# shaunliewsmu/ai-laryngeal-video-based-classifier

Hardware: AMD Instinct MI355X
Metric: clips/sec fwd ViViT-B 32x224^2 bf16 (higher is better)
Workload: dtype bf16; 1 GPU; ViViT-B/16x2 forward, 32x224x224 clips, batch 8 per GPU (BASELINE configs[1]); model=ViViT-B/16x2 (joint space-time, 12L, d768, 12H, 3137 tokens), global_batch=8, seq_len=3137, parallelism=dp1, streams=2, hip_graph=True

## Files before the change

ai-laryngeal-video-based-classifier_amd/_lib.py:

```python
from __future__ import annotations

import ctypes
import os
import re

import torch

from .build import LIB_PATH, INCLUDE

_lib = None

c_i64 = ctypes.c_int64
c_int = ctypes.c_int
c_f = ctypes.c_float
c_p = ctypes.c_void_p

SIGNATURES = {
    "vc_version": ([], ctypes.c_char_p),
    "vc_last_error": ([], ctypes.c_char_p),
    "vc_frame_gather": ([c_p, c_i64, c_i64, c_i64, c_i64, c_i64, c_p, c_i64, c_int, c_f, c_f, c_p, c_p], c_int),
    "vc_tubelet_im2col": ([c_p, c_i64, c_i64, c_i64, c_i64, c_i64, c_int, c_int, c_int, c_p, c_i64, c_p], c_int),
    "vc_patch_im2col": ([c_p, c_i64, c_i64, c_i64, c_i64, c_i64, c_int, c_int, c_int, c_int, c_int, c_p, c_i64, c_p],
                        c_int),
    "vc_layernorm_f32": ([c_p, c_i64, c_i64, c_i64, c_p, c_p, c_f, c_p, c_i64, c_p], c_int),
    "vc_gemm_bf16": ([c_p, c_i64, c_p, c_i64, c_i64, c_i64, c_i64, c_p, c_int, c_p, c_i64, c_p, c_i64,
                      c_i64, c_i64, c_i64, c_p], c_int),
    "vc_gemm_bf16_cfg": ([c_p, c_i64, c_p, c_i64, c_i64, c_i64, c_i64, c_p, c_int, c_p, c_i64, c_p, c_i64,
                          c_i64, c_i64, c_i64, c_int, c_p], c_int),
    "vc_layernorm_f32_bf16": ([c_p, c_i64, c_i64, c_i64, c_p, c_p, c_f, c_p, c_i64, c_p], c_int),
    "vc_attention_fwd": ([c_p, c_i64, c_i64, c_i64, c_i64, c_i64, c_f, c_int, c_p, c_i64, c_p], c_int),
    "vc_attention_fwd_rebase_always": ([c_p, c_i64, c_i64, c_i64, c_i64, c_f, c_p, c_i64, c_p], c_int),
    "vc_patch_im2col_h16": ([c_p, c_i64, c_i64, c_i64, c_i64, c_i64, c_int, c_int, c_int, c_int, c_int, c_int, c_p,
                             c_i64, c_p], c_int),
    "vc_gemm_pick": ([c_i64, c_i64, c_i64, c_int, c_i64, c_i64, c_p], c_int),
    "vc_gemm_h16_wrap": ([c_p, c_i64, c_i64, c_p, c_i64, c_i64, c_i64, c_i64, c_p, c_int, c_p, c_i64, c_p, c_i64,
                          c_i64, c_i64, c_i64, c_int, c_p], c_int),
    "vc_patch_im2col_split_h16": ([c_p, c_i64, c_i64, c_i64, c_i64, c_i64, c_int, c_int, c_int, c_int, c_int, c_int,
                                   c_p, c_i64, c_p], c_int),
    "vc_gemm_h16": ([c_p, c_i64, c_p, c_i64, c_i64, c_i64, c_i64, c_p, c_int, c_p, c_i64, c_p, c_i64,
                     c_i64, c_i64, c_i64, c_int, c_int, c_p], c_int),
    "vc_layernorm_f32_h16": ([c_p, c_i64, c_i64, c_i64, c_p, c_p, c_f, c_int, c_p, c_i64, c_p], c_int),
    "vc_attention_fwd_h16": ([c_p, c_i64, c_i64, c_i64, c_i64, c_i64, c_f, c_int, c_int, c_p, c_i64, c_p], c_int),
    "vc_spin": ([c_i64, c_i64, c_p], c_int),
    "vc_cls_init": ([c_p, c_p, c_p, c_i64, c_i64, c_i64, c_i64, c_p], c_int),
    "vc_cls_head": ([c_p, c_i64, c_i64, c_i64, c_i64, c_p, c_p, c_f, c_p, c_p, c_i64, c_p, c_p], c_int),
    "vc_temporal_attention": ([c_p, c_i64, c_i64, c_i64, c_i64, c_i64, c_i64, c_f, c_int, c_p, c_i64, c_p], c_int),
    "vc_window_attention3d": ([c_p, c_i64, c_i64, c_i64, c_i64, c_i64, c_i64, c_i64, c_int, c_int, c_int, c_int, c_int,
                               c_int, c_p, c_i64, c_p, c_i64, c_p], c_int),
    "vc_window_attention3d_mb": ([c_p, c_i64, c_i64, c_i64, c_i64, c_i64, c_i64, c_i64, c_int, c_int, c_int, c_int, c_int,
                               c_int, c_p, c_i64, c_p, c_i64, c_p], c_int),
    "vc_window_attention3d_lse": ([c_p, c_i64, c_i64, c_i64, c_i64, c_i64, c_i64, c_i64, c_int, c_int, c_int, c_int,
                                   c_int, c_int, c_p, c_i64, c_p, c_i64, c_p, c_p], c_int),
    "vc_window_attention3d_bwd": ([c_p, c_i64, c_p, c_i64, c_p, c_i64, c_p, c_i64, c_i64, c_i64, c_i64, c_i64, c_i64,
                                   c_int, c_int, c_int, c_int, c_int, c_int, c_int, c_int, c_int, c_p, c_p, c_i64,
                                   c_p, c_p], c_int),
    "vc_patch_merge_layernorm": ([c_p, c_i64, c_i64, c_i64, c_i64, c_i64, c_i64, c_p, c_p, c_f, c_p, c_i64, c_p], c_int),
    "vc_pool_head": ([c_p, c_i64, c_i64, c_i64, c_i64, c_p, c_p, c_f, c_p, c_p, c_i64, c_p, c_p, c_p], c_int),
    "vc_pool_head_pooled": ([c_p, c_i64, c_i64, c_i64, c_i64, c_p, c_p, c_f, c_p, c_p, c_i64, c_p, c_p, c_p, c_p],
                            c_int),
    "vc_pool_head_bwd": ([c_p, c_p, c_p, c_i64, c_i64, c_i64, c_f, c_p, c_p, c_p, c_p], c_int),
    "vc_conv3d_im2col": ([c_p, c_i64, c_int, c_i64, c_i64, c_i64, c_i64, c_i64, c_p, c_p, c_p, c_p, c_i64, c_p], c_int),
    "vc_conv3d_gemm_bf16": ([c_p, c_i64, c_i64, c_i64, c_i64, c_i64, c_i64, c_p, c_p, c_p, c_p, c_p, c_i64, c_i64,
                             c_p, c_int, c_p, c_i64, c_p, c_i64, c_p], c_int),
    "vc_conv3d_gemm_bf16_ring": ([c_p, c_i64, c_i64, c_i64, c_i64, c_i64, c_i64, c_p, c_p, c_p, c_p, c_p, c_i64, c_i64,
                                  c_p, c_int, c_p, c_i64, c_p, c_i64, c_int, c_p], c_int),
    "vc_conv3d_gemm_bf16_cfg": ([c_p, c_i64, c_i64, c_i64, c_i64, c_i64, c_i64, c_p, c_p, c_p, c_p, c_p, c_i64, c_i64,
                                 c_p, c_int, c_p, c_i64, c_p, c_i64, c_int, c_int, c_p], c_int),
    "vc_conv3d_stem_pack": ([c_p, c_i64, c_i64, c_i64, c_i64, c_i64, c_p, c_p, c_p], c_int),
    "vc_conv3d_stem_gemm_bf16": ([c_p, c_i64, c_i64, c_i64, c_i64, c_p, c_p, c_p, c_p, c_p, c_i64, c_i64, c_p, c_int,
                                  c_p, c_i64, c_p], c_int),
    "vc_maxpool3d": ([c_p, c_i64, c_i64, c_i64, c_i64, c_i64, c_i64, c_p, c_p, c_p, c_p, c_i64, c_p], c_int),
    "vc_avgpool_head": ([c_p, c_i64, c_i64, c_i64, c_i64, c_i64, c_i64, c_p, c_p, c_p, c_i64, c_p, c_p, c_p], c_int),
    "vc_col2im_cl": ([c_p, c_i64, c_i64, c_i64, c_i64, c_i64, c_i64, c_p, c_p, c_p, c_p, c_i64, c_p], c_int),
    "vc_maxpool3d_bwd": ([c_p, c_i64, c_p, c_int, c_i64, c_i64, c_i64, c_i64, c_i64, c_i64, c_p, c_p, c_p, c_p, c_i64,
                          c_p], c_int),
    "vc_batchnorm_train_fwd": ([c_p, c_i64, c_i64, c_i64, c_p, c_p, c_f, c_f, c_p, c_p, c_p, c_int, c_i64, c_int, c_p,
                                c_i64, c_p, c_p, c_i64, c_p], c_int),
    "vc_batchnorm_train_bwd": ([c_p, c_i64, c_i64, c_i64, c_p, c_p, c_p, c_i64, c_p, c_i64, c_int, c_p, c_i64, c_p,
# ... 81 lines not shown
```

ai-laryngeal-video-based-classifier_amd/ops.py:

```python
from __future__ import annotations

import torch

from . import _lib

EPI = {"bias": 0, "bias_gelu_tanh": 1, "bias_gelu_erf": 2, "bias_resid_f32": 3, "embed_f32": 4, "bias_f32": 5,
       "bias_relu": 6, "bias_resid_relu": 7, "bias_add_f32": 8, "bias_gelu_tanh_save": 9, "dgelu_tanh": 10}
GATHER_KIND = {"u8": 0, "f32": 1, "bf16": 2}


def _dev(*ts):
    for t in ts:
        if not isinstance(t, torch.Tensor) or t.device.type != "cuda":
            raise _lib.VclipError("vclip ops need CUDA(HIP) tensors; there is no CPU path")


def _stream(t: torch.Tensor) -> int:
    return torch.cuda.current_stream(t.device).cuda_stream


def _p(t):
    return t.data_ptr()


# ... 286 lines not shown
    return out


def layernorm_f32(x: torch.Tensor, gamma: torch.Tensor, beta: torch.Tensor, eps: float, out: torch.Tensor,
                  m: int | None = None) -> torch.Tensor:
    _dev(x, gamma, beta, out)
    M = x.shape[0] if m is None else m
    D = gamma.numel()
    _need(x.dtype == torch.float32 and out.dtype == torch.float32 and x.stride(1) == 1 and out.stride(1) == 1,
          "layernorm_f32 dtypes")
    _need(beta.numel() == D and x.shape[1] >= D and out.shape[1] >= D and x.shape[0] >= M and out.shape[0] >= M,
          "layernorm_f32 shapes")
    _lib.call("vc_layernorm_f32", _p(x), x.stride(0), M, D, _p(gamma), _p(beta), eps, _p(out), out.stride(0), _stream(x))
    return out


LOG2E = 1.4426950408889634


def attention(qkv: torch.Tensor, B: int, S: int, H: int, scale: float, out: torch.Tensor,
              q_prescaled: bool = False) -> torch.Tensor:
    _dev(qkv, out)
    _need(qkv.dtype in H16 and out.dtype == qkv.dtype and qkv.stride(1) == 1 and out.stride(1) == 1,
          "attention dtypes/layout")
    _need(qkv.shape[1] >= 3 * H * 64 and out.shape[1] >= H * 64, "attention columns")
    _need(qkv.shape[0] >= (B - 1) * S + (S + 63) // 64 * 64, "attention: qkv needs row padding to a 64-key tile")
    _need(out.shape[0] >= B * S, "attention out rows")
    if qkv.dtype == torch.float16:
        _lib.call("vc_attention_fwd_h16", _p(qkv), qkv.stride(0), B, S, H, 64, scale, int(bool(q_prescaled)), ELEM_F16,
                  _p(out), out.stride(0), _stream(qkv))
    else:
        _lib.call("vc_attention_fwd", _p(qkv), qkv.stride(0), B, S, H, 64, scale, int(bool(q_prescaled)), _p(out),
                  out.stride(0), _stream(qkv))
    return out


def spin(iters: int, device, blocks: int = 1) -> None:
    _lib.call("vc_spin", int(iters), int(blocks), torch.cuda.current_stream(device).cuda_stream)


def cls_init(cls: torch.Tensor, pos: torch.Tensor, x: torch.Tensor, B: int, S: int) -> torch.Tensor:
    _dev(cls, pos, x)
    D = cls.numel()
    _need(x.dtype == torch.float32 and x.shape[0] >= B * S and x.shape[1] >= D, "cls_init x")
    _lib.call("vc_cls_init", _p(cls), _p(pos), _p(x), x.stride(0), B, S, D, _stream(x))
    return x


def cls_head(x: torch.Tensor, B: int, S: int, gamma, beta, eps: float, wc: torch.Tensor, bc: torch.Tensor,
             out: torch.Tensor | None = None) -> torch.Tensor:
    _dev(x, gamma, beta, wc, bc)
    D = gamma.numel()
    nl = wc.shape[0]
    _need(wc.dtype == torch.float32 and wc.is_contiguous() and wc.shape[1] == D, "cls_head weight f32 [nl, D]")
    if out is None:
        out = torch.empty((B, nl), dtype=torch.float32, device=x.device)
    _lib.call("vc_cls_head", _p(x), x.stride(0), B, S, D, _p(gamma), _p(beta), eps, _p(wc), _p(bc), nl, _p(out),
              _stream(x))
    return out


def temporal_attention(qkv: torch.Tensor, B: int, P: int, T: int, H: int, scale: float, out: torch.Tensor,
                       q_prescaled: bool = False) -> torch.Tensor:
    _dev(qkv, out)
    _need(qkv.dtype == torch.bfloat16 and out.dtype == torch.bfloat16 and qkv.stride(1) == 1 and out.stride(1) == 1,
          "temporal_attention dtypes/layout")
# ... 763 lines not shown
```

ai-laryngeal-video-based-classifier_amd/vivit.py:

```python
from __future__ import annotations

import functools
import json
import math
from collections import OrderedDict

import numpy as np
import torch

from . import ops, streams
from .streams import GraphReplay
from .vivit_train import FlatLayout, TrainEngine, VivitTrainFn
from .weights import vivit_param_shapes


class VivitConfig:

    defaults = dict(image_size=224, num_frames=32, tubelet_size=[2, 16, 16], num_channels=3, hidden_size=768,
                    num_hidden_layers=12, num_attention_heads=12, intermediate_size=3072, hidden_act="gelu_fast",
                    hidden_dropout_prob=0.0, attention_probs_dropout_prob=0.0, initializer_range=0.02,
                    layer_norm_eps=1e-6, qkv_bias=True, model_type="vivit")

    def __init__(self, **kw):
        d = dict(self.defaults)
# ... 52 lines not shown
    def __init__(self, config: VivitConfig):
        super().__init__()
        self.config = config
        c = config
        if c.hidden_size // c.num_attention_heads != 64:
            raise ValueError("libvclip attention supports head_dim 64 only")
        self.params = torch.nn.ParameterDict()
        shapes = vivit_param_shapes(c.as_shape_cfg())
        self._names = list(shapes.keys())
        for name, shape in shapes.items():
            self.params[name.replace(".", "__")] = torch.nn.Parameter(torch.zeros(shape))
        self._layout = FlatLayout(c, shapes)
        self._flat = None
        self._gflat = None
        self._gscratch = None
        self._engine = None
        self.grad_ready_hooks = []
        self._packed = None
        self._ws = {}
        self._ws_used = []
        self._streams = None
        self.concurrent_streams = None
        self.stream_priorities = None
        self.split_sizes = None
        self.last_streams = 1
        self.kernel_events = None
        self.graph_replay = False
        self._graphs = GraphReplay()
        self.gemm_cfg = {}
        self.rows = "pad"
        self.compute_dtype = torch.bfloat16
        self.precise_layers = 0
        self.precise_ops = ("embed_w", "qkv")

    def hf_state_dict(self):
        return OrderedDict((n, self.params[n.replace(".", "__")]) for n in self._names)

    def state_dict(self, *a, **k):
        return OrderedDict((n, p.detach()) for n, p in self.hf_state_dict().items())

    def load_state_dict(self, sd, strict: bool = True):
        from .checkpoint import convert_state_dict
        sd = convert_state_dict(sd)
        missing = [n for n in self._names if n not in sd]
        unexpected = [k for k in sd if k not in self._names]
        if strict and (missing or unexpected):
            raise KeyError(f"load_state_dict: missing={missing[:5]} unexpected={unexpected[:5]}")
        with torch.no_grad():
            for n in self._names:
                if n in sd:
                    v = sd[n]
                    v = torch.as_tensor(np.asarray(v)) if not isinstance(v, torch.Tensor) else v
                    self.params[n.replace(".", "__")].copy_(v.reshape(self.params[n.replace(".", "__")].shape))
        self._packed = None
        return missing, unexpected

    def P(self, name):
        return self.params[name.replace(".", "__")]

    def _param_list(self):
        return [self.P(n) for n in self._names]

    def _apply(self, fn, *args, **kwargs):
        out = super()._apply(fn, *args, **kwargs)
        self._flat = self._gflat = self._gscratch = self._engine = None
        self._packed = None
# ... 143 lines not shown

    def geometry(self, B):
        c = self.config
        kt, kh, kw = c.tubelet_size
        npatch = (c.num_frames // kt) * (c.image_size // kh) * (c.image_size // kw)
        S = npatch + 1
        Mpad = _round_up(B * S + 128, 256)
        Memb = _round_up(B * npatch, 128)
        return npatch, S, Mpad, Memb

    def _workspace(self, B, device, part: int = 0):
        key = (B, str(device), part, self.compute_dtype, self.precise_layers > 0)
        if key in self._ws:
            ws = self._ws[key]
            if not any(w is ws for w in self._ws_used):
                self._ws_used.append(ws)
            return ws
        if len(self._ws) >= 8:
            self._ws = {}
        c = self.config
        D, I = c.hidden_size, c.intermediate_size
        kt, kh, kw = c.tubelet_size
        npatch, S, Mpad, Memb = self.geometry(B)
        bf = self.compute_dtype
        z = lambda *s, dt=bf: torch.zeros(s, dtype=dt, device=device)
        Kemb = c.num_channels * kt * kh * kw
        precise = self.precise_layers > 0 and bf == torch.float16
        if precise:
            Memb = _round_up(B * npatch, 256)
            Xe = z(Mpad + 256, D, dt=torch.float32)
        else:
            Xe = z(Mpad, D, dt=torch.float32)
        ws = dict(A_emb=z(Memb, Kemb), X=Xe[:Mpad], X_emb=Xe, Y=z(Mpad, D),
                  QKV=z(Mpad, 3 * D), O=z(Mpad, D), Hd=z(Mpad, I), logits=z(B, c.num_labels, dt=torch.float32))
        if precise:
            ws["A_emb_split"] = z(Memb, 2 * Kemb)
        self._ws[key] = ws
        self._ws_used.append(ws)
        return ws

    def forward(self, pixel_values: torch.Tensor = None, labels: torch.Tensor = None, **kw):
        if pixel_values is None:
            raise ValueError("pixel_values required")
        if pixel_values.device.type != "cuda":
            raise RuntimeError("VivitForVideoClassification (vclip_amd) runs on the GPU only: move pixel_values "
                               "to cuda (the reference's `.to(device)`, trainer.py:92)")
        x = pixel_values.contiguous().float() if pixel_values.dtype != torch.float32 else pixel_values.contiguous()
        params = self._param_list()
        if self.training and torch.is_grad_enabled() and any(p.requires_grad for p in params):
            logits = VivitTrainFn.apply(self, x, *params)
        else:
            with torch.no_grad():
                logits = self.forward_logits(x).clone()
        loss = None
        if labels is not None:
            loss = torch.nn.functional.cross_entropy(logits, labels.to(logits.device))
        return ClassifierOutput(logits, loss)

    @torch.no_grad()
    def forward_logits(self, pix: torch.Tensor) -> torch.Tensor:
        c = self.config
        B, T, C, H, W = pix.shape
        if T != c.num_frames or H != c.image_size or W != c.image_size or C != c.num_channels:
            raise ValueError(f"pixel_values {tuple(pix.shape)} do not match config "
                             f"(T={c.num_frames}, C={c.num_channels}, {c.image_size}^2)")
        if (self.graph_replay and self.kernel_events is None and not streams.serial()
                and not torch.cuda.is_current_stream_capturing()):
            key = (pix.data_ptr(), tuple(pix.shape), tuple(pix.stride()), pix.dtype, self.concurrent_streams,
                   self.compute_dtype, self._weights_version(),
                   tuple(sorted((k, tuple(v) if isinstance(v, list) else v) for k, v in self.gemm_cfg.items())), self.rows,
                   self.precise_layers, tuple(sorted(self.precise_ops)),
                   None if self.split_sizes is None else tuple(self.split_sizes),
                   None if self.stream_priorities is None else tuple(self.stream_priorities))
            return self._graphs.run(key, pix, self._forward_eager, keep=lambda: (self._packed, tuple(self._ws_used)))
        return self._forward_eager(pix)

    def _forward_eager(self, pix: torch.Tensor) -> torch.Tensor:
        self._ws_used = []
        c = self.config
        B = pix.shape[0]
        ns = self.concurrent_streams or 1
        ns = max(1, min(int(ns), B))
        self.last_streams = ns
        if ns == 1:
            self.last_split = [B]
            return self._forward_part(pix, 0)
        dev = pix.device
        key = (B, str(dev), "logits")
        if key not in self._ws:
            self._ws[key] = torch.zeros(B, c.num_labels, dtype=torch.float32, device=dev)
        logits = self._ws[key]
        cur = torch.cuda.current_stream(dev)
        self._pack(dev)
        bounds = streams.split_bounds(B, ns, self.split_sizes if self.split_sizes is not None
                                      else SPLIT_DEFAULT.get((B, ns)))
        self.last_split = [bounds[i + 1] - bounds[i] for i in range(ns)]
        if streams.serial():
            for i in range(ns):
                self._forward_part(pix[bounds[i]:bounds[i + 1]], i, out=logits[bounds[i]:bounds[i + 1]])
            return logits
        def go(sts):
            for st in sts:
                pix.record_stream(st)
            streams.fork_parts(sts, cur, [lambda i=i: self._forward_part(pix[bounds[i]:bounds[i + 1]], i,
                                                                          out=logits[bounds[i]:bounds[i + 1]])
                                          for i in range(ns)])

        self._streams = streams.part_streams(self, (B, ns, str(dev), tuple(bounds), self.compute_dtype), ns, go,
                                             dev, self.stream_priorities)
        go(self._streams)
        return logits

    def _forward_part(self, pix: torch.Tensor, part: int, out=None) -> torch.Tensor:
        c = self.config
        B = pix.shape[0]
        pk = self._pack(pix.device)
        ws = self._workspace(B, pix.device, part)
        D = c.hidden_size
        npatch, S, Mpad, Memb = self.geometry(B)
        kt_, kh_, kw_ = c.tubelet_size
        eps = c.layer_norm_eps
        X, Y, QKV, O, Hd = ws["X"], ws["Y"], ws["QKV"], ws["O"], ws["Hd"]
        ev = self.kernel_events

        def run(name, fn, *args, **kw):
            if ev is None or (not isinstance(ev, dict) and name != "attention"):
                return fn(*args, **kw)
            e0, e1 = torch.cuda.Event(enable_timing=True), torch.cuda.Event(enable_timing=True)
            e0.record()
            r = fn(*args, **kw)
            e1.record()
            (ev.setdefault(name, []) if isinstance(ev, dict) else ev).append((e0, e1))
            return r

        M = B * S
        I = c.intermediate_size
        Kemb = c.num_channels * kt_ * kh_ * kw_
        T_, H_ = c.num_frames, c.image_size
        ln_bytes = M * D * (4 + 2)
        tm = ops.timed
        if "A_emb_split" in ws and "w_emb_split" in pk and "embed_w" in pk["pops"]:
            run("im2col", tm, "im2col_kernel", "im2col", B * (T_ * c.num_channels * H_ * H_ * 4 + npatch * Kemb * 2),
                "byte", ops.tubelet_im2col, pix, c.tubelet_size, ws["A_emb"])
            run("embed", ops.gemm_wrap, ws["A_emb"], Kemb, pk["w_emb_split"], pk["b_emb"], "embed_f32", ws["X_emb"],
                aux=pk["pos"][1:], group=npatch, group_stride=S, group_offset=1, m=ws["A_emb"].shape[0],
                flop=2.0 * B * npatch * D * Kemb, op="embed")
        elif "A_emb_split" in ws and "w_emb_split" in pk:
            run("im2col", tm, "im2col_kernel", "im2col", B * (T_ * c.num_channels * H_ * H_ * 4 + npatch * Kemb * 4),
                "byte", ops.patch_im2col_split, pix, c.tubelet_size, ws["A_emb_split"])
            run("embed", ops.gemm_wrap, ws["A_emb_split"], 2 * Kemb, pk["w_emb_split"], pk["b_emb"], "embed_f32",
                ws["X_emb"], aux=pk["pos"][1:], group=npatch, group_stride=S, group_offset=1,
                m=ws["A_emb_split"].shape[0],
                flop=2.0 * B * npatch * D * Kemb, op="embed")
        else:
            run("im2col", tm, "im2col_kernel", "im2col", B * (T_ * c.num_channels * H_ * H_ * 4 + npatch * Kemb * 2),
                "byte", ops.tubelet_im2col, pix, c.tubelet_size, ws["A_emb"])
            run("embed", ops.gemm, ws["A_emb"], pk["w_emb"], pk["b_emb"], "embed_f32", X, aux=pk["pos"][1:],
                group=npatch, group_stride=S, group_offset=1, m=Memb, flop=2.0 * B * npatch * D * Kemb, op="embed")
        ops.cls_init(pk["cls"], pk["pos"], X, B, S)
        act = "bias_gelu_tanh" if c.hidden_act in ("gelu_fast", "gelu_pytorch_tanh", "gelu_new") else "bias_gelu_erf"
        scale = 1.0 / math.sqrt(D // c.num_attention_heads)
        qkv_gemm = fc2_gemm = ops.gemm
        gc = self.gemm_cfg
        tight = self.rows == "tight"

        def rows(name):
            cfg = gc.get(name)
            if isinstance(cfg, (list, tuple)):
                cfg = cfg[part]
            if not tight:
                return None, -1 if cfg is None else cfg
            h = 128 if cfg in (5, 7, 21) else 256
            return _round_up(B * S, h), -1 if cfg is None else cfg

        m_ln = B * S if tight else None
        (m_qkv, c_qkv), (m_o, c_o), (m_1, c_1), (m_2, c_2) = rows("qkv"), rows("o_proj"), rows("fc1"), rows("fc2")
        Hn = c.num_attention_heads
        attn_flop = 4.0 * S * S * (D // Hn) * Hn * B
        for L in pk["layers"]:
            sp = L.get("split", {})
            run("layernorm", tm, "layernorm_kernel", "layernorm", ln_bytes, "byte", ops.layernorm, X, L["ln1_g"],
                L["ln1_b"], eps, Y, m=m_ln)
            if "w_qkv" in sp:
                run("qkv", ops.gemm_wrap, Y, D, sp["w_qkv"], L["b_qkv"], "bias", QKV, flop=2.0 * M * 3 * D * D, op="qkv")
            else:
                run("qkv", qkv_gemm, Y, L["w_qkv"], L["b_qkv"], "bias", QKV, m=m_qkv, cfg=c_qkv,
                    flop=2.0 * M * 3 * D * D, op="qkv")
            run("attention", tm, "attn_fwd_d64_kernel", "attention", attn_flop, "flop", ops.attention, QKV, B, S, Hn,
                scale, O, q_prescaled=True)
            if "w_o" in sp:
                run("o_proj", ops.gemm_wrap, O, D, sp["w_o"], L["b_o"], "bias_resid_f32", X, flop=2.0 * M * D * D,
                    op="o_proj")
            else:
                run("o_proj", ops.gemm, O, L["w_o"], L["b_o"], "bias_resid_f32", X, m=m_o, cfg=c_o,
                    flop=2.0 * M * D * D, op="o_proj")
            run("layernorm", tm, "layernorm_kernel", "layernorm", ln_bytes, "byte", ops.layernorm, X, L["ln2_g"],
                L["ln2_b"], eps, Y, m=m_ln)
            if "w_1" in sp:
                run("fc1", ops.gemm_wrap, Y, D, sp["w_1"], L["b_1"], act, Hd, flop=2.0 * M * I * D, op="fc1")
            else:
                run("fc1", ops.gemm, Y, L["w_1"], L["b_1"], act, Hd, m=m_1, cfg=c_1, flop=2.0 * M * I * D, op="fc1")
            if "w_2" in sp:
                run("fc2", ops.gemm_wrap, Hd, I, sp["w_2"], L["b_2"], "bias_resid_f32", X, flop=2.0 * M * D * I,
                    op="fc2")
            else:
                run("fc2", fc2_gemm, Hd, L["w_2"], L["b_2"], "bias_resid_f32", X, m=m_2, cfg=c_2,
                    flop=2.0 * M * D * I, op="fc2")
        return ops.cls_head(X, B, S, pk["lnf_g"], pk["lnf_b"], eps, pk["w_cls"], pk["b_cls"],
                            out=ws["logits"] if out is None else out)


def create_model(model_name="google/vivit-b-16x2-kinetics400", num_classes=2, class_labels=None, num_frames=32,
                 device="cuda", logger=None, weights_seed: int = 0):
    class_labels = class_labels or ["non-referral", "referral"]
    id2label = {i: l for i, l in enumerate(class_labels)}
    cfg = VivitConfig(num_frames=num_frames, id2label=id2label, label2id={l: i for i, l in id2label.items()})
    if logger:
        logger.info(f"Creating ViViT model {model_name} (num_frames={num_frames}, labels={class_labels}) on {device}")
    model = VivitForVideoClassification(cfg)
    from .weights import make_vivit_weights
# ... 4 lines not shown
```

include/vclip.h:

```cpp
#ifndef VCLIP_H_
#define VCLIP_H_

#include <stdint.h>
#include <hip/hip_runtime_api.h>

#ifdef __cplusplus
extern "C" {
#endif

#define VC_ERR_INVALID_ARG (-1)
#define VC_ERR_UNSUPPORTED (-2)

const char* vc_version(void);

const char* vc_last_error(void);

#define VC_GATHER_U8_NHWC   0
#define VC_GATHER_F32_NCHW  1
#define VC_GATHER_BF16_NCHW 2

int vc_frame_gather(const uint8_t* frames, int64_t nclips, int64_t F, int64_t H, int64_t W, int64_t C,
                    const int64_t* idx, int64_t T, int out_kind, float scale, float shift,
                    void* out, hipStream_t stream);

// ... 51 lines not shown

int vc_gemm_pick(int64_t M, int64_t N, int64_t K, int epilogue, int64_t ldo, int64_t ldaux, const void* aux);

int vc_gemm_h16(const uint16_t* A, int64_t lda, const uint16_t* W, int64_t ldw,
                int64_t M, int64_t N, int64_t K, const float* bias, int epilogue,
                void* out, int64_t ldo, const float* aux, int64_t ldaux,
                int64_t G, int64_t group_stride, int64_t group_offset, int elem, int cfg, hipStream_t stream);

int vc_gemm_h16_wrap(const uint16_t* A, int64_t lda, int64_t ka, const uint16_t* W, int64_t ldw, int64_t M,
                     int64_t N, int64_t K, const float* bias, int epilogue, void* out, int64_t ldo, const float* aux,
                     int64_t ldaux, int64_t G, int64_t group_stride, int64_t group_offset, int elem,
                     hipStream_t stream);
int vc_patch_im2col_split_h16(const float* pixel_values, int64_t B, int64_t T, int64_t C, int64_t H, int64_t W,
                              int kt, int kh, int kw, int token_order, int layout, int elem, uint16_t* A, int64_t lda,
                              hipStream_t stream);

int vc_layernorm_f32_h16(const float* x, int64_t ldx, int64_t M, int64_t D, const float* gamma, const float* beta,
                         float eps, int elem, uint16_t* y, int64_t ldy, hipStream_t stream);

int vc_attention_fwd_h16(const uint16_t* qkv, int64_t ld, int64_t B, int64_t S, int64_t H, int64_t head_dim,
                         float scale, int q_prescaled, int elem, uint16_t* out, int64_t ldo, hipStream_t stream);

int vc_layernorm_f32(const float* x, int64_t ldx, int64_t M, int64_t D, const float* gamma, const float* beta,
                     float eps, float* y, int64_t ldy, hipStream_t stream);

int vc_spin(int64_t iters, int64_t blocks, hipStream_t stream);

int vc_cls_init(const float* cls, const float* pos, float* x, int64_t ldx, int64_t B, int64_t S, int64_t D,
                hipStream_t stream);

int vc_cls_head(const float* x, int64_t ldx, int64_t B, int64_t S, int64_t D,
                const float* gamma, const float* beta, float eps,
                const float* Wc, const float* bc, int64_t num_labels, float* logits, hipStream_t stream);


int vc_resample_u8(const uint8_t* src, int64_t N, int64_t H, int64_t W, int64_t C, int axis, int64_t out_size,
                   const int* bounds, const int* coeffs, int64_t ksize, uint8_t* dst, hipStream_t stream);

int vc_resize_linear_u8(const uint8_t* src, int64_t N, int64_t H, int64_t W, int64_t C, int64_t h, int64_t w,
                        const int* tables, int64_t xlim, int area2x, uint8_t* dst, hipStream_t stream);

int vc_video_transform(const uint8_t* frames, int64_t nclips, int64_t F, int64_t H, int64_t W, const int64_t* idx,
                       int64_t T, int64_t resize_h, int64_t resize_w, int64_t top, int64_t left, int64_t crop_h,
                       int64_t crop_w, const float* scale3, const float* shift3, int layout, int out_bf16, void* out,
                       hipStream_t stream);

int vc_video_transform_clips(const uint8_t* frames, int64_t nclips, int64_t F, int64_t H, int64_t W, const int64_t* idx,
                             int64_t T, const int* clip_params, int64_t crop_h, int64_t crop_w, const float* scale3,
                             const float* shift3, int layout, int out_bf16, void* out, hipStream_t stream);


int vc_temporal_attention(const uint16_t* qkv, int64_t ld, int64_t B, int64_t P, int64_t T, int64_t H,
                          int64_t head_dim, float scale, int q_prescaled, uint16_t* out, int64_t ldo,
                          hipStream_t stream);

#define VC_DIVIDED_TEMPORAL_TO_SPATIAL 0
#define VC_DIVIDED_SPATIAL_TO_MLP      1
int vc_divided_add_layernorm(float* x, int64_t ldx, const uint16_t* y, int64_t ldy, int64_t B, int64_t P, int64_t T,
                             int64_t D, const float* gamma, const float* beta, float eps, int mode, uint16_t* h,
                             int64_t ldh, hipStream_t stream);

#define VC_CONV_IN_NCTHW_F32 0
#define VC_CONV_IN_CL_BF16   1
int vc_conv3d_im2col(const void* x, int64_t ldx, int input_kind, int64_t B, int64_t T, int64_t H, int64_t W,
                     int64_t C, const int* kernel, const int* stride, const int* pad, uint16_t* A, int64_t lda,
                     hipStream_t stream);
// ... 183 lines not shown
```

Baseline: 1011 clips/s.

## Compute only the CLS token in the final transformer layer at inference

In eval mode the last encoder layer now computes attention only for each clip's CLS query. It uses a split-K CLS attention kernel plus a combine step, then runs o_proj, LayerNorm+fc1 and fc2 on just the B CLS rows with new skinny GEMM kernels. This removes the full-sequence attention and MLP work in the final layer, whose other token outputs are never consumed. It adds new kernels, a work buffer and a graph key flag, and it depends on the head reading only the CLS row.

Result: faster. 1075 clips/s (median of 6 runs) (+6.3%).

```diff
diff --git a/ai-laryngeal-video-based-classifier_amd/_lib.py b/ai-laryngeal-video-based-classifier_amd/_lib.py
--- a/ai-laryngeal-video-based-classifier_amd/_lib.py
+++ b/ai-laryngeal-video-based-classifier_amd/_lib.py
@@ -44,6 +44,9 @@
     "vc_spin": ([c_i64, c_i64, c_p], c_int),
     "vc_cls_init": ([c_p, c_p, c_p, c_i64, c_i64, c_i64, c_i64, c_p], c_int),
     "vc_cls_head": ([c_p, c_i64, c_i64, c_i64, c_i64, c_p, c_p, c_f, c_p, c_p, c_i64, c_p, c_p], c_int),
+    "vc_cls_attention": ([c_p, c_i64, c_i64, c_i64, c_i64, c_i64, c_int, c_p, c_i64, c_p, c_i64, c_p], c_int),
+    "vc_skinny_gemm": ([c_p, c_i64, c_p, c_p, c_f, c_p, c_i64, c_i64, c_i64, c_i64, c_p, c_int, c_int, c_p, c_i64,
+                        c_p], c_int),
     "vc_temporal_attention": ([c_p, c_i64, c_i64, c_i64, c_i64, c_i64, c_i64, c_f, c_int, c_p, c_i64, c_p], c_int),
     "vc_window_attention3d": ([c_p, c_i64, c_i64, c_i64, c_i64, c_i64, c_i64, c_i64, c_int, c_int, c_int, c_int, c_int,
                                c_int, c_p, c_i64, c_p, c_i64, c_p], c_int),
diff --git a/ai-laryngeal-video-based-classifier_amd/csrc/cls_tail.hip b/ai-laryngeal-video-based-classifier_amd/csrc/cls_tail.hip
--- /dev/null
+++ b/ai-laryngeal-video-based-classifier_amd/csrc/cls_tail.hip
@@ -0,0 +1,329 @@
+#include "common.hpp"
+
+namespace vc {
+
+constexpr int kClsSplit = VC_CLS_ATTN_SPLIT;
+constexpr int kClsPart = 66;
+
+template <int ET>
+__global__ void __launch_bounds__(256) cls_attn_kernel(const uint16_t* __restrict__ qkv, int64_t ld, int S, int H,
+                                                       int nsplit, float* __restrict__ part) {
+    __shared__ float red[4];
+    __shared__ float redl[4];
+    __shared__ float redo[4][64];
+    const int split = blockIdx.x, h = blockIdx.y, b = blockIdx.z;
+    const int tid = threadIdx.x, lane = tid & 63, wave = tid >> 6;
+    const int sub = tid & 7;
+    const int kslot = tid >> 3;
+    const int64_t row0 = (int64_t)b * S;
+    const int HD = H * 64;
+    const uint16_t* qp = qkv + row0 * ld + h * 64 + sub * 8;
+    const uint16_t* kbase = qkv + HD + h * 64 + sub * 8;
+    const uint16_t* vbase = qkv + 2 * HD + h * 64 + sub * 8;
+    const v8s q8 = *reinterpret_cast<const v8s*>(qp);
+    constexpr int NP = kClsSplit / 32;
+    v8s k8[NP], v8[NP];
+    const int key0 = split * kClsSplit + kslot;
+#pragma unroll
+    for (int i = 0; i < NP; ++i) {
+        const int key = key0 + i * 32;
+        const int64_t r = row0 + (key < S ? key : S - 1);
+        k8[i] = *reinterpret_cast<const v8s*>(kbase + r * ld);
+        v8[i] = *reinterpret_cast<const v8s*>(vbase + r * ld);
+    }
+    float q[8];
+#pragma unroll
+    for (int e = 0; e < 8; ++e) q[e] = from16<ET>((unsigned short)q8[e]);
+    float s[NP];
+    float m = -INFINITY;
+#pragma unroll
+    for (int i = 0; i < NP; ++i) {
+        float d = 0.f;
+#pragma unroll
+        for (int e = 0; e < 8; ++e) d = __builtin_fmaf(q[e], from16<ET>((unsigned short)k8[i][e]), d);
+        d = group_sum<8>(d);
+        s[i] = key0 + i * 32 < S ? d : -INFINITY;
+        m = fmaxf(m, s[i]);
+    }
+#pragma unroll
+    for (int o = 32; o >= 8; o >>= 1) m = fmaxf(m, __shfl_xor(m, o, 64));
+    if (lane == 0) red[wave] = m;
+    __syncthreads();
+    m = fmaxf(fmaxf(red[0], red[1]), fmaxf(red[2], red[3]));
+    float l = 0.f;
+    float o[8] = {0.f, 0.f, 0.f, 0.f, 0.f, 0.f, 0.f, 0.f};
+#pragma unroll
+    for (int i = 0; i < NP; ++i) {
+        const float p = key0 + i * 32 < S ? __builtin_amdgcn_exp2f(s[i] - m) : 0.f;
+        l += p;
+#pragma unroll
+        for (int e = 0; e < 8; ++e) o[e] = __builtin_fmaf(p, from16<ET>((unsigned short)v8[i][e]), o[e]);
+    }
+#pragma unroll
+    for (int sh = 8; sh <= 32; sh <<= 1) {
+        l += __shfl_xor(l, sh, 64);
+#pragma unroll
+        for (int e = 0; e < 8; ++e) o[e] += __shfl_xor(o[e], sh, 64);
+    }
+    if (lane < 8) {
+#pragma unroll
+        for (int e = 0; e < 8; ++e) redo[wave][lane * 8 + e] = o[e];
+        if (lane == 0) redl[wave] = l;
+    }
+    __syncthreads();
+    if (tid < 64) {
+        float* dst = part + ((int64_t)(b * H + h) * nsplit + split) * kClsPart;
+        dst[2 + tid] = ((redo[0][tid] + redo[1][tid]) + redo[2][tid]) + redo[3][tid];
+        if (tid == 0) {
+            dst[0] = m;
+            dst[1] = ((redl[0] + redl[1]) + redl[2]) + redl[3];
+        }
+    }
+}
+
+template <int ET>
+__global__ void __launch_bounds__(64) cls_attn_combine_kernel(const float* __restrict__ part, int S, int H, int nsplit,
+                                                              uint16_t* __restrict__ out, int64_t ldo) {
+    const int h = blockIdx.x, b = blockIdx.y, d = threadIdx.x;
+    const float* p = part + (int64_t)(b * H + h) * nsplit * kClsPart;
+    float m = -INFINITY;
+    for (int i = d; i < nsplit; i += 64) m = fmaxf(m, p[i * kClsPart]);
+#pragma unroll
+    for (int o = 32; o > 0; o >>= 1) m = fmaxf(m, __shfl_xor(m, o, 64));
+    float l = 0.f;
+    for (int i = d; i < nsplit; i += 64) l = __builtin_fmaf(__builtin_amdgcn_exp2f(p[i * kClsPart] - m), p[i * kClsPart + 1], l);
+    l = wave_sum(l);
+    float o = 0.f;
+    for (int i0 = 0; i0 < nsplit; i0 += 4) {
+        float mv[4], ov[4];
+#pragma unroll
+        for (int u = 0; u < 4; ++u) {
+            const int i = i0 + u < nsplit ? i0 + u : nsplit - 1;
+            mv[u] = p[i * kClsPart];
+            ov[u] = p[i * kClsPart + 2 + d];
+        }
+#pragma unroll
+        for (int u = 0; u < 4; ++u)
+            if (i0 + u < nsplit) o = __builtin_fmaf(__builtin_amdgcn_exp2f(mv[u] - m), ov[u], o);
+    }
+    out[(int64_t)b * S * ldo + h * 64 + d] = to16<ET>(o / l);
+}
+
+constexpr int kSkinnyRows = 8;
+constexpr int kSkinnyFrags = VC_SKINNY_MAX_K / 512;
+constexpr int kLnRegV = 4;
+
+template <int ET, bool LN>
+__global__ void __launch_bounds__(256) skinny_gemm_kernel(const void* __restrict__ a_, int64_t lda, const float* __restrict__ ln_g,
+                                                          const float* __restrict__ ln_b, float eps,
+                                                          const uint16_t* __restrict__ w, int64_t ldw, int M, int N, int K,
+                                                          const float* __restrict__ bias, int epilogue, void* out_,
+                                                          int64_t ldo) {
+    extern __shared__ __attribute__((aligned(16))) char smem[];
+    uint16_t* As = reinterpret_cast<uint16_t*>(smem);
+    const int tid = threadIdx.x, lane = tid & 63, wave = tid >> 6;
+    const int r0 = blockIdx.y * kSkinnyRows;
+    const int mc = M - r0 < kSkinnyRows ? M - r0 : kSkinnyRows;
+    const int n = blockIdx.x * 4 + wave;
+    v8s wreg[kSkinnyFrags];
+    {
+        const uint16_t* wr = w + (int64_t)(n < N ? n : N - 1) * ldw;
+#pragma unroll
+        for (int j = 0; j < kSkinnyFrags; ++j) {
+            const int k = (j * 64 + lane) * 8;
+            if (j * 512 < K) wreg[j] = *reinterpret_cast<const v8s*>(wr + (k < K ? k : 0));
+        }
+    }
+    if constexpr (LN) {
+#pragma clang fp contract(off)
+        const float* a = reinterpret_cast<const float*>(a_);
+        const int K4 = K >> 2;
+        const float4* g4 = reinterpret_cast<const float4*>(ln_g);
+        const float4* b4 = reinterpret_cast<const float4*>(ln_b);
+        if (K4 <= 64 * kLnRegV) {
+            float4 v[2][kLnRegV], gg[kLnRegV], bb[kLnRegV];
+#pragma unroll
+            for (int rr = 0; rr < 2; ++rr) {
+                const int r = wave + 4 * rr;
+                const float4* xr = reinterpret_cast<const float4*>(a + (int64_t)(r0 + (r < mc ? r : 0)) * lda);
+#pragma unroll
+                for (int i = 0; i < kLnRegV; ++i) v[rr][i] = xr[i * 64 + lane < K4 ? i * 64 + lane : 0];
+            }
+#pragma unroll
+            for (int i = 0; i < kLnRegV; ++i) {
+                gg[i] = g4[i * 64 + lane < K4 ? i * 64 + lane : 0];
+                bb[i] = b4[i * 64 + lane < K4 ? i * 64 + lane : 0];
+            }
+#pragma unroll
+            for (int rr = 0; rr < 2; ++rr) {
+                const int r = wave + 4 * rr;
+                float s = 0.f;
+#pragma unroll
+                for (int i = 0; i < kLnRegV; ++i)
+                    if (i * 64 + lane < K4) s += (v[rr][i].x + v[rr][i].y) + (v[rr][i].z + v[rr][i].w);
+                const float mean = wave_sum(s) * (1.0f / K);
+                float q = 0.f;
+#pragma unroll
+                for (int i = 0; i < kLnRegV; ++i)
+                    if (i * 64 + lane < K4) {
+                        const float x0 = v[rr][i].x - mean, x1 = v[rr][i].y - mean, x2 = v[rr][i].z - mean, x3 = v[rr][i].w - mean;
+                        q += (x0 * x0 + x1 * x1) + (x2 * x2 + x3 * x3);
+                    }
+                const float rstd = rsqrtf(wave_sum(q) * (1.0f / K) + eps);
+#pragma unroll
+                for (int i = 0; i < kLnRegV; ++i)
+                    if (i * 64 + lane < K4) {
+                        uint2 o = make_uint2(0u, 0u);
+                        if (r < mc) {
+                            o.x = pack2<ET>((v[rr][i].x - mean) * rstd * gg[i].x + bb[i].x, (v[rr][i].y - mean) * rstd * gg[i].y + bb[i].y);
+                            o.y = pack2<ET>((v[rr][i].z - mean) * rstd * gg[i].z + bb[i].z, (v[rr][i].w - mean) * rstd * gg[i].w + bb[i].w);
+                        }
+                        *reinterpret_cast<uint2*>(As + r * K + (i * 64 + lane) * 4) = o;
+                    }
+            }
+        } else {
+            for (int r = wave; r < kSkinnyRows; r += 4) {
+                if (r >= mc) {
+                    for (int i = lane; i < K4; i += 64) *reinterpret_cast<uint2*>(As + r * K + i * 4) = make_uint2(0u, 0u);
+                    continue;
+                }
+                const float4* xr = reinterpret_cast<const float4*>(a + (int64_t)(r0 + r) * lda);
+                float s = 0.f;
+                for (int i = lane; i < K4; i += 64) {
+                    const float4 x = xr[i];
+                    s += (x.x + x.y) + (x.z + x.w);
+                }
+                const float mean = wave_sum(s) * (1.0f / K);
+                float q = 0.f;
+                for (int i = lane; i < K4; i += 64) {
+                    const float4 x = xr[i];
+                    const float x0 = x.x - mean, x1 = x.y - mean, x2 = x.z - mean, x3 = x.w - mean;
+                    q += (x0 * x0 + x1 * x1) + (x2 * x2 + x3 * x3);
+                }
+                const float rstd = rsqrtf(wave_sum(q) * (1.0f / K) + eps);
+                for (int i = lane; i < K4; i += 64) {
+                    const float4 x = xr[i], gg = g4[i], bb = b4[i];
+                    uint2 o;
+                    o.x = pack2<ET>((x.x - mean) * rstd * gg.x + bb.x, (x.y - mean) * rstd * gg.y + bb.y);
+                    o.y = pack2<ET>((x.z - mean) * rstd * gg.z + bb.z, (x.w - mean) * rstd * gg.w + bb.w);
+                    *reinterpret_cast<uint2*>(As + r * K + i * 4) = o;
+                }
+            }
+        }
+    } else {
+        const uint16_t* a = reinterpret_cast<const uint16_t*>(a_);
+        const int K8 = K >> 3;
+        for (int i = tid; i < kSkinnyRows * K8; i += 256) {
+            const int r = i / K8, c = i - r * K8;
+            v4u v = {0u, 0u, 0u, 0u};
+            if (r < mc) v = *reinterpret_cast<const v4u*>(a + (int64_t)(r0 + r) * lda + c * 8);
+            *reinterpret_cast<v4u*>(As + r * K + c * 8) = v;
+        }
+    }
+    __syncthreads();
+    if (n >= N) return;
+    float acc[kSkinnyRows];
+#pragma unroll
+    for (int r = 0; r < kSkinnyRows; ++r) acc[r] = 0.f;
+#pragma unroll
+    for (int j = 0; j < kSkinnyFrags; ++j) {
+        const int k = (j * 64 + lane) * 8;
+        if (k < K) {
+            float wf[8];
+#pragma unroll
+            for (int e = 0; e < 8; ++e) wf[e] = from16<ET>((unsigned short)wreg[j][e]);
+#pragma unroll
+            for (int r = 0; r < kSkinnyRows; ++r) {
+                const v8s a8 = *reinterpret_cast<const v8s*>(As + r * K + k);
+#pragma unroll
+                for (int e = 0; e < 8; ++e) acc[r] = __builtin_fmaf(from16<ET>((unsigned short)a8[e]), wf[e], acc[r]);
+            }
+        }
+    }
+    float mine = 0.f;
+#pragma unroll
+    for (int r = 0; r < kSkinnyRows; ++r) {
+        const float t = wave_sum(acc[r]);
+        if (lane == r) mine = t;
+    }
+    if (lane < mc) {
+        const float v = mine + bias[n];
+        const int64_t o = (int64_t)(r0 + lane) * ldo + n;
+        if (epilogue == VC_EPI_BIAS_RESID_F32) {
+            float* out = reinterpret_cast<float*>(out_);
+            out[o] += v;
+        } else {
+            uint16_t* out = reinterpret_cast<uint16_t*>(out_);
+            out[o] = to16<ET>(epilogue == VC_EPI_BIAS_GELU_TANH ? gelu_tanh(v) : epilogue == VC_EPI_BIAS_GELU_ERF ? gelu_erf(v) : v);
+        }
+    }
+}
+
+template <int ET>
+static int cls_attention(const uint16_t* qkv, int64_t ld, int64_t B, int64_t S, int64_t H, float* work, uint16_t* out,
+                         int64_t ldo, hipStream_t stream) {
+    const int nsplit = (int)((S + kClsSplit - 1) / kClsSplit);
+    cls_attn_kernel<ET><<<dim3((unsigned)nsplit, (unsigned)H, (unsigned)B), 256, 0, stream>>>(qkv, ld, (int)S, (int)H, nsplit, work);
+    int rc = check_launch("vc_cls_attention");
+    if (rc) return rc;
+    cls_attn_combine_kernel<ET><<<dim3((unsigned)H, (unsigned)B), 64, 0, stream>>>(work, (int)S, (int)H, nsplit, out, ldo);
+    return check_launch("vc_cls_attention (combine)");
+}
+
+template <int ET>
+static int skinny_gemm(const void* a, int64_t lda, const float* g, const float* b, float eps, const uint16_t* w, int64_t ldw,
+                       int64_t M, int64_t N, int64_t K, const float* bias, int epilogue, void* out, int64_t ldo,
+                       hipStream_t stream) {
+    const dim3 grid((unsigned)((N + 3) / 4), (unsigned)((M + kSkinnyRows - 1) / kSkinnyRows));
+    const size_t lds = (size_t)kSkinnyRows * K * 2;
+    if (g)
+        skinny_gemm_kernel<ET, true><<<grid, 256, lds, stream>>>(a, lda, g, b, eps, w, ldw, (int)M, (int)N, (int)K, bias, epilogue, out, ldo);
+    else
+        skinny_gemm_kernel<ET, false><<<grid, 256, lds, stream>>>(a, lda, g, b, eps, w, ldw, (int)M, (int)N, (int)K, bias, epilogue, out, ldo);
+    return check_launch("vc_skinny_gemm");
+}
+
+}
+
+using namespace vc;
+
+extern "C" {
+
+int vc_cls_attention(const uint16_t* qkv, int64_t ld, int64_t B, int64_t S, int64_t H, int64_t head_dim, int elem,
+                     float* work, int64_t work_elems, uint16_t* out, int64_t ldo, hipStream_t stream) {
+    if (!qkv || !work || !out) return fail(VC_ERR_INVALID_ARG, "vc_cls_attention: null pointer");
+    if (head_dim != 64) return fail(VC_ERR_UNSUPPORTED, "vc_cls_attention: head_dim must be 64");
+    if (elem != VC_ELEM_BF16 && elem != VC_ELEM_F16) return fail(VC_ERR_INVALID_ARG, "vc_cls_attention: bad elem");
+    if (B <= 0 || S <= 0 || H <= 0 || B > 65535 || H > 65535 || B * S >= (int64_t)1 << 31)
+        return fail(VC_ERR_INVALID_ARG, "vc_cls_attention: bad B / S / H");
+    if (ld < 3 * H * 64 || ld % 8 || ((uintptr_t)qkv & 15)) return fail(VC_ERR_INVALID_ARG, "vc_cls_attention: qkv needs ld >= 3*H*64, ld % 8 == 0 and 16-byte alignment");
+    if (ldo < H * 64) return fail(VC_ERR_INVALID_ARG, "vc_cls_attention: ldo < H*64");
+    const int64_t nsplit = (S + kClsSplit - 1) / kClsSplit;
+    if (work_elems < B * H * nsplit * kClsPart) return fail(VC_ERR_INVALID_ARG, "vc_cls_attention: work buffer too small");
+    if (elem == VC_ELEM_F16) return cls_attention<VC_ELEM_F16>(qkv, ld, B, S, H, work, out, ldo, stream);
+    return cls_attention<VC_ELEM_BF16>(qkv, ld, B, S, H, work, out, ldo, stream);
+}
+
+int vc_skinny_gemm(const void* A, int64_t lda, const float* ln_gamma, const float* ln_beta, float ln_eps,
+                   const uint16_t* W, int64_t ldw, int64_t M, int64_t N, int64_t K, const float* bias, int epilogue,
+                   int elem, void* out, int64_t ldo, hipStream_t stream) {
+    if (!A || !W || !bias || !out) return fail(VC_ERR_INVALID_ARG, "vc_skinny_gemm: null pointer");
+    if ((ln_gamma == nullptr) != (ln_beta == nullptr)) return fail(VC_ERR_INVALID_ARG, "vc_skinny_gemm: gamma and beta go together");
+    if (elem != VC_ELEM_BF16 && elem != VC_ELEM_F16) return fail(VC_ERR_INVALID_ARG, "vc_skinny_gemm: bad elem");
+    if (epilogue != VC_EPI_BIAS_BF16 && epilogue != VC_EPI_BIAS_GELU_TANH && epilogue != VC_EPI_BIAS_GELU_ERF &&
+        epilogue != VC_EPI_BIAS_RESID_F32)
+        return fail(VC_ERR_UNSUPPORTED, "vc_skinny_gemm: epilogue must be bias, bias + gelu or bias + f32 residual");
+    if (M <= 0 || N <= 0 || K <= 0 || M > 8 * 65535 || N >= (int64_t)1 << 31) return fail(VC_ERR_INVALID_ARG, "vc_skinny_gemm: bad M / N / K");
+    if (K % 8 || K > VC_SKINNY_MAX_K) return fail(VC_ERR_UNSUPPORTED, "vc_skinny_gemm: K must be a multiple of 8, at most VC_SKINNY_MAX_K");
+    if (ldw < K || ldw % 8 || ((uintptr_t)W & 15)) return fail(VC_ERR_INVALID_ARG, "vc_skinny_gemm: W needs ldw >= K, ldw % 8 == 0 and 16-byte alignment");
+    if (ln_gamma) {
+        if (lda % 4 || (((uintptr_t)A | (uintptr_t)ln_gamma | (uintptr_t)ln_beta) & 15))
+            return fail(VC_ERR_INVALID_ARG, "vc_skinny_gemm: f32 A, gamma and beta need 16-byte alignment and lda % 4 == 0");
+    } else if (lda % 8 || ((uintptr_t)A & 15))
+        return fail(VC_ERR_INVALID_ARG, "vc_skinny_gemm: 16-bit A needs 16-byte alignment and lda % 8 == 0");
+    if (elem == VC_ELEM_F16)
+        return skinny_gemm<VC_ELEM_F16>(A, lda, ln_gamma, ln_beta, ln_eps, W, ldw, M, N, K, bias, epilogue, out, ldo, stream);
+    return skinny_gemm<VC_ELEM_BF16>(A, lda, ln_gamma, ln_beta, ln_eps, W, ldw, M, N, K, bias, epilogue, out, ldo, stream);
+}
+
+}
diff --git a/ai-laryngeal-video-based-classifier_amd/ops.py b/ai-laryngeal-video-based-classifier_amd/ops.py
--- a/ai-laryngeal-video-based-classifier_amd/ops.py
+++ b/ai-laryngeal-video-based-classifier_amd/ops.py
@@ -342,6 +342,57 @@
     else:
         _lib.call("vc_attention_fwd", _p(qkv), qkv.stride(0), B, S, H, 64, scale, int(bool(q_prescaled)), _p(out),
                   out.stride(0), _stream(qkv))
+    return out
+
+
+ATTN_SHORT_MAX_S = 256
+CLS_ATTN_SPLIT = 256
+SKINNY_MAX_K = 4096
+
+
+def cls_attention_work(B: int, S: int, H: int, device) -> torch.Tensor:
+    return torch.zeros(B * H * ((S + CLS_ATTN_SPLIT - 1) // CLS_ATTN_SPLIT) * 66, dtype=torch.float32, device=device)
+
+
+def cls_attention(qkv: torch.Tensor, B: int, S: int, H: int, work: torch.Tensor, out: torch.Tensor) -> torch.Tensor:
+    _dev(qkv, work, out)
+    _need(qkv.dtype in H16 and out.dtype == qkv.dtype and qkv.stride(1) == 1 and out.stride(1) == 1,
+          "cls_attention dtypes/layout")
+    _need(qkv.shape[1] >= 3 * H * 64 and out.shape[1] >= H * 64, "cls_attention columns")
+    _need(qkv.shape[0] >= B * S and out.shape[0] >= (B - 1) * S + 1, "cls_attention rows")
+    _need(work.dtype == torch.float32 and work.is_contiguous(), "cls_attention work: contiguous f32")
+    _lib.call("vc_cls_attention", _p(qkv), qkv.stride(0), B, S, H, 64, ELEM_F16 if qkv.dtype == torch.float16 else 0,
+              _p(work), work.numel(), _p(out), out.stride(0), _stream(qkv))
+    return out
+
+
+def skinny_gemm_takes(K: int) -> bool:
+    return K % 8 == 0 and 0 < K <= SKINNY_MAX_K
+
+
+def skinny_gemm(a: torch.Tensor, w: torch.Tensor, bias: torch.Tensor, epilogue: str, out: torch.Tensor,
+                ln: tuple | None = None) -> torch.Tensor:
+    _dev(a, w, bias, out)
+    M, K = a.shape
+    N = w.shape[0]
+    _need(w.dtype in H16 and w.dim() == 2 and w.shape[1] == K and w.stride(1) == 1 and bias.dtype == torch.float32 and
+          bias.numel() == N and bias.is_contiguous(), "skinny_gemm: w 16-bit [N, K], bias f32 [N]")
+    _need(a.dim() == 2 and a.stride(1) == 1 and out.dim() == 2 and out.stride(1) == 1 and out.shape[0] >= M and
+          out.shape[1] >= N, "skinny_gemm: a [M, K], out [>= M, >= N], unit column strides")
+    _need(epilogue in ("bias", "bias_gelu_tanh", "bias_gelu_erf", "bias_resid_f32"), f"skinny_gemm: epilogue {epilogue}")
+    _need(out.dtype == (torch.float32 if epilogue == "bias_resid_f32" else w.dtype), "skinny_gemm out dtype")
+    if ln is None:
+        _need(a.dtype == w.dtype, "skinny_gemm: a must have w's type")
+        g = b = None
+        eps = 0.0
+    else:
+        g, b, eps = ln
+        _dev(g, b)
+        _need(a.dtype == torch.float32 and g.dtype == torch.float32 and b.dtype == torch.float32 and g.numel() == K and
+              b.numel() == K and g.is_contiguous() and b.is_contiguous(), "skinny_gemm: LayerNorm prologue on f32 rows")
+    _lib.call("vc_skinny_gemm", _p(a), a.stride(0), None if g is None else _p(g), None if b is None else _p(b), eps,
+              _p(w), w.stride(0), M, N, K, _p(bias), EPI[epilogue], ELEM_F16 if w.dtype == torch.float16 else 0, _p(out),
+              out.stride(0), _stream(a))
     return out
 
 
diff --git a/ai-laryngeal-video-based-classifier_amd/vivit.py b/ai-laryngeal-video-based-classifier_amd/vivit.py
--- a/ai-laryngeal-video-based-classifier_amd/vivit.py
+++ b/ai-laryngeal-video-based-classifier_amd/vivit.py
@@ -108,6 +108,7 @@
         self.compute_dtype = torch.bfloat16
         self.precise_layers = 0
         self.precise_ops = ("embed_w", "qkv")
+        self.cls_only_last_layer = True
 
     def hf_state_dict(self):
         return OrderedDict((n, self.params[n.replace(".", "__")]) for n in self._names)
@@ -317,7 +318,8 @@
         else:
             Xe = z(Mpad, D, dt=torch.float32)
         ws = dict(A_emb=z(Memb, Kemb), X=Xe[:Mpad], X_emb=Xe, Y=z(Mpad, D),
-                  QKV=z(Mpad, 3 * D), O=z(Mpad, D), Hd=z(Mpad, I), logits=z(B, c.num_labels, dt=torch.float32))
+                  QKV=z(Mpad, 3 * D), O=z(Mpad, D), Hd=z(Mpad, I), logits=z(B, c.num_labels, dt=torch.float32),
+                  cls_work=ops.cls_attention_work(B, S, c.num_attention_heads, device), Hc=z(B, I))
         if precise:
             ws["A_emb_split"] = z(Memb, 2 * Kemb)
         self._ws[key] = ws
@@ -356,9 +358,13 @@
                    tuple(sorted((k, tuple(v) if isinstance(v, list) else v) for k, v in self.gemm_cfg.items())), self.rows,
                    self.precise_layers, tuple(sorted(self.precise_ops)),
                    None if self.split_sizes is None else tuple(self.split_sizes),
-                   None if self.stream_priorities is None else tuple(self.stream_priorities))
+                   None if self.stream_priorities is None else tuple(self.stream_priorities),
+                   self._cls_only())
             return self._graphs.run(key, pix, self._forward_eager, keep=lambda: (self._packed, tuple(self._ws_used)))
         return self._forward_eager(pix)
+
+    def _cls_only(self) -> bool:
+        return bool(self.cls_only_last_layer) and not self.training
 
     def _forward_eager(self, pix: torch.Tensor) -> torch.Tensor:
         self._ws_used = []
@@ -369,7 +375,7 @@
         self.last_streams = ns
         if ns == 1:
             self.last_split = [B]
-            return self._forward_part(pix, 0)
+            return self._forward_part(pix, 0, cls_only=self._cls_only())
         dev = pix.device
         key = (B, str(dev), "logits")
         if key not in self._ws:
@@ -380,15 +386,18 @@
         bounds = streams.split_bounds(B, ns, self.split_sizes if self.split_sizes is not None
                                       else SPLIT_DEFAULT.get((B, ns)))
         self.last_split = [bounds[i + 1] - bounds[i] for i in range(ns)]
+        cls_only = self._cls_only()
         if streams.serial():
             for i in range(ns):
-                self._forward_part(pix[bounds[i]:bounds[i + 1]], i, out=logits[bounds[i]:bounds[i + 1]])
+                self._forward_part(pix[bounds[i]:bounds[i + 1]], i, out=logits[bounds[i]:bounds[i + 1]],
+                                   cls_only=cls_only)
             return logits
         def go(sts):
             for st in sts:
                 pix.record_stream(st)
             streams.fork_parts(sts, cur, [lambda i=i: self._forward_part(pix[bounds[i]:bounds[i + 1]], i,
-                                                                          out=logits[bounds[i]:bounds[i + 1]])
+                                                                          out=logits[bounds[i]:bounds[i + 1]],
+                                                                          cls_only=cls_only)
                                           for i in range(ns)])
 
         self._streams = streams.part_streams(self, (B, ns, str(dev), tuple(bounds), self.compute_dtype), ns, go,
@@ -396,7 +405,7 @@
         go(self._streams)
         return logits
 
-    def _forward_part(self, pix: torch.Tensor, part: int, out=None) -> torch.Tensor:
+    def _forward_part(self, pix: torch.Tensor, part: int, out=None, cls_only: bool = False) -> torch.Tensor:
         c = self.config
         B = pix.shape[0]
         pk = self._pack(pix.device)
@@ -462,7 +471,11 @@
         (m_qkv, c_qkv), (m_o, c_o), (m_1, c_1), (m_2, c_2) = rows("qkv"), rows("o_proj"), rows("fc1"), rows("fc2")
         Hn = c.num_attention_heads
         attn_flop = 4.0 * S * S * (D // Hn) * Hn * B
-        for L in pk["layers"]:
+        n_full = len(pk["layers"])
+        if (cls_only and n_full and "split" not in pk["layers"][-1] and D // Hn == 64
+                and ops.skinny_gemm_takes(D) and ops.skinny_gemm_takes(I)):
+            n_full -= 1
+        for li, L in enumerate(pk["layers"]):
             sp = L.get("split", {})
             run("layernorm", tm, "layernorm_kernel", "layernorm", ln_bytes, "byte", ops.layernorm, X, L["ln1_g"],
                 L["ln1_b"], eps, Y, m=m_ln)
@@ -471,6 +484,22 @@
             else:
                 run("qkv", qkv_gemm, Y, L["w_qkv"], L["b_qkv"], "bias", QKV, m=m_qkv, cfg=c_qkv,
                     flop=2.0 * M * 3 * D * D, op="qkv")
+            if li >= n_full:
+                Xc, Oc, Hc = X[:M:S], O[:M:S], ws["Hc"]
+                es = Y.element_size()
+                if S <= ops.ATTN_SHORT_MAX_S:
+                    run("attention", tm, "attn_fwd_d64_kernel", "attention", attn_flop, "flop", ops.attention, QKV, B,
+                        S, Hn, scale, O, q_prescaled=True)
+                else:
+                    run("cls_attention", tm, "cls_attn_kernel", "cls_attention", B * (2 * S + 2) * D * es, "byte",
+                        ops.cls_attention, QKV, B, S, Hn, ws["cls_work"], O)
+                run("cls_o_proj", tm, "skinny_gemm_kernel", "cls_o_proj", D * D * es, "byte", ops.skinny_gemm, Oc,
+                    L["w_o"], L["b_o"], "bias_resid_f32", Xc)
+                run("cls_fc1", tm, "skinny_gemm_kernel", "cls_fc1", I * D * es, "byte", ops.skinny_gemm, Xc, L["w_1"],
+                    L["b_1"], act, Hc, ln=(L["ln2_g"], L["ln2_b"], eps))
+                run("cls_fc2", tm, "skinny_gemm_kernel", "cls_fc2", D * I * es, "byte", ops.skinny_gemm, Hc, L["w_2"],
+                    L["b_2"], "bias_resid_f32", Xc)
+                continue
             run("attention", tm, "attn_fwd_d64_kernel", "attention", attn_flop, "flop", ops.attention, QKV, B, S, Hn,
                 scale, O, q_prescaled=True)
             if "w_o" in sp:
diff --git a/include/vclip.h b/include/vclip.h
--- a/include/vclip.h
+++ b/include/vclip.h
@@ -107,6 +107,17 @@
 int vc_cls_head(const float* x, int64_t ldx, int64_t B, int64_t S, int64_t D,
                 const float* gamma, const float* beta, float eps,
                 const float* Wc, const float* bc, int64_t num_labels, float* logits, hipStream_t stream);
+
+
+#define VC_CLS_ATTN_SPLIT 256
+#define VC_SKINNY_MAX_K 4096
+
+int vc_cls_attention(const uint16_t* qkv, int64_t ld, int64_t B, int64_t S, int64_t H, int64_t head_dim, int elem,
+                     float* work, int64_t work_elems, uint16_t* out, int64_t ldo, hipStream_t stream);
+
+int vc_skinny_gemm(const void* A, int64_t lda, const float* ln_gamma, const float* ln_beta, float ln_eps,
+                   const uint16_t* W, int64_t ldw, int64_t M, int64_t N, int64_t K, const float* bias, int epilogue,
+                   int elem, void* out, int64_t ldo, hipStream_t stream);
 
 
 int vc_resample_u8(const uint8_t* src, int64_t N, int64_t H, int64_t W, int64_t C, int axis, int64_t out_size,
```
